# jepsen-io/maelstrom

Hardware: NVIDIA B200
Metric: simulated msgs/sec (broadcast, 4096 nodes) (higher is better)
Workload: dtype int64

## Files before the change

maelstrom_b200/csrc/ms_device.cuh:

```cuda
#pragma once
#include <stdint.h>
#include "../../include/maelstrom_b200.h"

#if defined(__CUDACC__)
#define MS_HD __host__ __device__ __forceinline__
#else
#define MS_HD inline
#endif

namespace msd {

constexpr int64_t  kTickNs   = 1000000;
constexpr uint32_t kInjector = 0xFFFFFFFFu;
constexpr uint8_t  kRemoved  = 0x80;

enum : uint32_t {
  E_NONE = 0, E_RING_OVERFLOW = 1, E_WINDOW_OVERFLOW = 2, E_JOURNAL_OVERFLOW = 3,
  E_INVALID_DEST = 4, E_HISTORY = 5, E_VALUE_RANGE = 6, E_MAIL_OVERFLOW = 7,
  E_CALENDAR_OVERFLOW = 8, E_ID_RANGE = 9, E_BARRIER = 10, E_SNAPSHOT = 11,
  E_RAFT_CAPACITY = 12, E_HISTORY_RING = 13
};

#ifndef MS_CLS0_NT
#define MS_CLS0_NT 64
// ... 53 lines not shown
  uint64_t ev_total, em_total;
};

struct NetParams {
  uint64_t loss_thresh;
  uint64_t exp_coeff;
  uint32_t dist;
  uint32_t mean_ms;
  uint32_t scale;
  uint32_t pair_active;
  uint32_t comp_active;
  uint32_t any_removed;
};

struct Params {
  DevState* st;
  NetParams* np;
  uint8_t*  kind;
  uint32_t* tail;
  uint32_t* limit;
  uint32_t* head;
  uint64_t* ep_born;
  uint4*    ring;
  uint32_t  ring_cap, ring_cap_s;
  uint32_t  n_ep, n_servers, n_inj_tickets, max_window, max_window_s;
  RoundMeta* rmeta;
  uint32_t* rt_em;
  uint32_t* rt_ev;
  uint64_t* rt_chunk;
  uint64_t* rt_cnt;
  uint64_t* phase_cycles;
  uint32_t  n_shards, shard_id;
  uint4*    ring_sh[8];
  uint32_t* tail_sh[8];
  uint32_t* head_sh[8];
  uint64_t* rt_cnt_sh[8];
  uint32_t* bar_sh[8];
  uint32_t  hist, hist_mask, t_max, n_classes;
  uint32_t  split_commit;
  uint64_t* cm_blk;
  uint32_t* cm_flags;
  uint32_t* cls_list;
  uint32_t  cls_cap[4];
  uint4*    jraw;
  uint4*    jbody;
  uint64_t  jmask;
// ... 196 lines not shown
```

maelstrom_b200/csrc/ms_engine.cu:

```cuda
#include <cuda_runtime.h>
#include <math.h>
#include <stdio.h>
#include <stdlib.h>
#include <string.h>

#include <algorithm>
#include <deque>
#include <mutex>
#include <new>
#include <string>
#include <unordered_map>
#include <vector>

#include "ms_device.cuh"
#include "ms_tree.h"
#include "ms_fressian.h"
#include "ms_json.h"

using namespace msd;

extern "C" {
cudaError_t msk_round_smem_attr(size_t bytes);
size_t msk_round_smem_bytes(uint32_t cap);
int msk_round_occupancy(int threads, size_t smem);
// ... 544 lines not shown
  if (cudaGetDeviceCount(&ndev) != cudaSuccess || ndev == 0) {
    set_err("no CUDA device: maelstrom_b200 has no CPU fallback");
    return MS_ERR_CUDA;
  }
  s->device = c.device;
  CK(cudaSetDevice(s->device));
  CK(cudaStreamCreateWithFlags(&s->stream, cudaStreamNonBlocking));
  for (int k = 0; k < 4; k++) CK(cudaStreamCreateWithFlags(&s->aux_streams[k], cudaStreamNonBlocking));
  for (int k = 0; k < 5; k++) CK(cudaEventCreateWithFlags(&s->aux_events[k], cudaEventDisableTiming));

  Params& P = s->P;
  memset(&P, 0, sizeof P);
  const uint32_t M = c.max_endpoints;
  int rc;
  if ((rc = s->dalloc(&P.st, 1))) return rc;
  if ((rc = s->dalloc(&P.np, 1))) return rc;
  if ((rc = s->dalloc(&P.kind, M))) return rc;
  if ((rc = s->dalloc(&P.tail, M))) return rc;
  if ((rc = s->dalloc(&P.limit, M))) return rc;
  if ((rc = s->dalloc(&P.head, M))) return rc;
  if ((rc = s->dalloc(&P.ep_born, M))) return rc;
  {
    void* ptr = nullptr;
    CK(cudaMalloc(&ptr, ((size_t)c.n_nodes * c.server_ring_cap + (size_t)(M - c.n_nodes) * c.ring_cap) * 48));
    s->allocs.push_back(ptr);
    P.ring = (uint4*)ptr;
  }
  P.ring_cap = c.ring_cap;
  P.ring_cap_s = c.server_ring_cap;
  P.n_servers = c.n_nodes;
  P.n_ep = c.n_nodes;
  P.n_inj_tickets = 8;
  P.max_window = c.max_window;
  P.max_window_s = c.server_max_window;
  s->use_graph = c.reserved[1] == 1;
  P.n_shards = c.n_shards;
  P.shard_id = c.shard_id;
  {
    P.t_max = M + P.n_inj_tickets;
    const uint32_t hist = history_rows(c.reserved[0], P.t_max);
    P.hist = hist;
    P.hist_mask = hist - 1;
    if ((rc = s->dalloc(&P.rmeta, hist))) return rc;
    if ((rc = s->dalloc(&P.rt_em, (size_t)hist * P.t_max))) return rc;
    if ((rc = s->dalloc(&P.rt_ev, (size_t)hist * P.t_max))) return rc;
    if ((rc = s->dalloc(&P.rt_chunk, (size_t)hist * P.t_max))) return rc;
    if ((rc = s->dalloc(&P.rt_cnt, (size_t)hist * P.t_max))) return rc;
// ... 1127 lines not shown
  out[0] = (uint64_t)r.state; out[1] = r.term; out[2] = (uint64_t)(r.voted_for + 1); out[3] = r.commit_index;
  out[4] = r.last_applied; out[5] = (uint64_t)(r.leader + 1); out[6] = r.log_size; out[7] = r.kv_size;
  return MS_OK;
}

int ms_counters(ms_sim* s, uint64_t out[8]) {
  std::lock_guard<std::mutex> g(s->mu);
  out[0] = s->hs.rounds_run;
  out[1] = s->hs.stats[2] + s->hs.stats[4];
  out[2] = s->hs.stats[3] + s->hs.stats[5];
  out[3] = s->launches;
  out[4] = s->hs.lost;
  out[5] = s->hs.part_drops;
  out[6] = s->hs.max_window_seen;
  out[7] = s->hs.fallback_sorts;
  return MS_OK;
}

struct ShardBlob {
  uint32_t magic, shard_id, n_shards, t_max;
  uint32_t max_endpoints, ring_cap, hist, pad;
  cudaIpcMemHandle_t ring, tail, head, rt_cnt, bar;
  cudaIpcMemHandle_t gs_snap, gs_tag;
};
static_assert(sizeof(ShardBlob) <= MS_SHARD_BLOB_BYTES, "blob too large");

int ms_shard_handles(ms_sim* s, void* blob_out) {
  std::lock_guard<std::mutex> g(s->mu);
  cudaSetDevice(s->device);
  ShardBlob b;
  memset(&b, 0, sizeof b);
  b.magic = 0x4253534Du;
  b.shard_id = s->P.shard_id; b.n_shards = s->P.n_shards; b.t_max = s->P.t_max;
  b.max_endpoints = s->cfg.max_endpoints; b.ring_cap = s->P.ring_cap ^ (s->P.ring_cap_s << 1); b.hist = s->P.hist;
  CK(cudaIpcGetMemHandle(&b.ring, s->P.ring));
  CK(cudaIpcGetMemHandle(&b.tail, s->P.tail));
  CK(cudaIpcGetMemHandle(&b.head, s->P.head));
  CK(cudaIpcGetMemHandle(&b.rt_cnt, s->P.rt_cnt));
  CK(cudaIpcGetMemHandle(&b.bar, s->P.bar_sh[s->P.shard_id]));
  if (s->P.gs_snap) {
    b.pad = 1;
    CK(cudaIpcGetMemHandle(&b.gs_snap, s->P.gs_snap));
    CK(cudaIpcGetMemHandle(&b.gs_tag, s->P.gs_tag));
  } else if (s->P.rf_heap) {
    b.pad = 2;
    CK(cudaIpcGetMemHandle(&b.gs_snap, s->P.rf_heap));
    CK(cudaIpcGetMemHandle(&b.gs_tag, s->P.rf_ext_off));
  }
  memset(blob_out, 0, MS_SHARD_BLOB_BYTES);
  memcpy(blob_out, &b, sizeof b);
  return MS_OK;
}

int ms_shard_connect(ms_sim* s, uint32_t peer, const void* blob) {
  std::lock_guard<std::mutex> g(s->mu);
  cudaSetDevice(s->device);
  ShardBlob b;
  memcpy(&b, blob, sizeof b);
  if (b.magic != 0x4253534Du || b.shard_id != peer || peer >= s->P.n_shards || b.n_shards != s->P.n_shards ||
      b.t_max != s->P.t_max || b.max_endpoints != s->cfg.max_endpoints || b.ring_cap != (s->P.ring_cap ^ (s->P.ring_cap_s << 1)) ||
      b.hist != s->P.hist) {
    set_err("ms_shard_connect: peer blob does not match this simulation's configuration");
    return MS_ERR_ARG;
  }
  if (peer == s->P.shard_id) return MS_OK;
  void* ptr = nullptr;
  CK(cudaIpcOpenMemHandle(&ptr, b.ring, cudaIpcMemLazyEnablePeerAccess));
  s->peer_ptrs.push_back(ptr); s->P.ring_sh[peer] = (uint4*)ptr;
  CK(cudaIpcOpenMemHandle(&ptr, b.tail, cudaIpcMemLazyEnablePeerAccess));
  s->peer_ptrs.push_back(ptr); s->P.tail_sh[peer] = (uint32_t*)ptr;
  CK(cudaIpcOpenMemHandle(&ptr, b.head, cudaIpcMemLazyEnablePeerAccess));
  s->peer_ptrs.push_back(ptr); s->P.head_sh[peer] = (uint32_t*)ptr;
  CK(cudaIpcOpenMemHandle(&ptr, b.rt_cnt, cudaIpcMemLazyEnablePeerAccess));
  s->peer_ptrs.push_back(ptr); s->P.rt_cnt_sh[peer] = (uint64_t*)ptr;
  CK(cudaIpcOpenMemHandle(&ptr, b.bar, cudaIpcMemLazyEnablePeerAccess));
  s->peer_ptrs.push_back(ptr); s->P.bar_sh[peer] = (uint32_t*)ptr;
  if ((b.pad == 1) != (s->P.gs_snap != nullptr) || (b.pad == 2) != (s->P.rf_heap != nullptr)) {
    set_err("ms_shard_connect: peer runs another workload");
    return MS_ERR_ARG;
  }
  if (b.pad == 2) {
    const size_t N = s->cfg.n_nodes;
    CK(cudaIpcOpenMemHandle(&ptr, b.gs_snap, cudaIpcMemLazyEnablePeerAccess));
    s->peer_ptrs.push_back(ptr); s->P.rf_heap_sh[peer] = (uint4*)ptr;
// ... 100 lines not shown
```

maelstrom_b200/csrc/ms_kernels.cu:

```cuda
#include <cuda_runtime.h>
#include <stdint.h>
#include "ms_device.cuh"

namespace msd {

#define FULL 0xFFFFFFFFu
#ifndef MS_EMUL
#define MS_LAUNCH(kern, grid, block, smem, stream, ...) kern<<<(grid), (block), (smem), (stream)>>>(__VA_ARGS__)
#endif
constexpr int MAXB = 64;
constexpr int MAXNB = 8;
constexpr uint64_t RECV_BIT = 1ull << 63;
constexpr uint32_t kResolvedTicket = 0xFFFFFFu;

__device__ __forceinline__ uint32_t ld_cg_u32(const uint32_t* p) { return __ldcg(p); }
__device__ __forceinline__ void st_v4(uint4* p, uint4 v) {
#ifdef MS_EMUL
  *p = v;
#else
  asm volatile("st.global.L1::no_allocate.v4.u32 [%0], {%1,%2,%3,%4};" ::"l"(p), "r"(v.x), "r"(v.y),
               "r"(v.z), "r"(v.w)
               : "memory");
#endif
}
// ... 23 lines not shown
}

__device__ __forceinline__ bool round_skipped(const Params& p, const DevState* st) {
  if (st->now >= st->stop_ns || st->error) return true;
  if (p.jlevel && !p.jdiscard) {
    const uint64_t raw_base = p.rmeta[(uint32_t)st->round & p.hist_mask].raw_base;
    if (p.n_shards <= 1 && raw_base - st->jraw_drained > ((p.jmask + 1) >> 1)) return true;
    if (st->round - st->drain_round + 2 >= p.hist) return true;
  }
  return false;
}

__device__ __forceinline__ uint32_t slot_tag(uint64_t round) { return 0x80000000u | (uint32_t)(round & 0x7FFFFFFFull); }

struct Rec {
  uint64_t round;
  uint32_t ticket, idx;
  uint32_t src, dest, msg_id, in_reply_to;
  uint32_t tf;
  uint32_t p0;
  uint64_t p1;
};

__device__ __forceinline__ void rec_store(uint4* slot, const Rec& r) {
  st_v4(slot + 0, make_uint4(r.idx, r.ticket, (uint32_t)r.round, (uint32_t)(r.round >> 32)));
  st_v4(slot + 1, make_uint4(r.src, r.dest, r.msg_id, r.in_reply_to));
  st_v4(slot + 2, make_uint4(r.tf, r.p0, (uint32_t)r.p1, (uint32_t)(r.p1 >> 32)));
}
__device__ __forceinline__ Rec rec_unpack(uint4 a, uint4 b, uint4 c) {
  Rec r;
  r.idx = a.x; r.ticket = a.y;
  r.round = (uint64_t)a.z | ((uint64_t)a.w << 32);
  r.src = b.x; r.dest = b.y; r.msg_id = b.z; r.in_reply_to = b.w;
  r.tf = c.x; r.p0 = c.y;
  r.p1 = (uint64_t)c.z | ((uint64_t)c.w << 32);
  return r;
}

__device__ __forceinline__ uint32_t ring_cap_of(const Params& p, uint32_t e) { return e < p.n_servers ? p.ring_cap_s : p.ring_cap; }
__device__ __forceinline__ size_t ring_base(const Params& p, uint32_t e) {
  return e < p.n_servers ? (size_t)e * p.ring_cap_s
                         : (size_t)p.n_servers * p.ring_cap_s + (size_t)(e - p.n_servers) * p.ring_cap;
}
__device__ __forceinline__ uint4* ring_slot(const Params& p, uint4* ring, uint32_t e, uint32_t pos) {
  return ring + (ring_base(p, e) + (pos & (ring_cap_of(p, e) - 1u))) * 3;
}

__device__ __forceinline__ uint64_t dense_base(const Params& p, DevState* st, uint64_t round, uint32_t ticket) {
  if (ticket == kResolvedTicket) return round << 32;
  const uint32_t row = (uint32_t)round & p.hist_mask;
  const RoundMeta* m = p.rmeta + row;
  if (m->round != round || ticket >= p.t_max) {
    latch_error(st, E_HISTORY, (uint32_t)round);
    return 0;
  }
  return m->id_base + p.rt_em[(size_t)row * p.t_max + ticket];
}

__device__ uint64_t block_excl_scan(uint64_t* a, int n, uint64_t* wtmp ) {
  const int nt = blockDim.x, tid = threadIdx.x, lane = tid & 31, warp = tid >> 5;
  const int c = (n + nt - 1) / nt;
  const int lo = min(tid * c, n), hi = min(lo + c, n);
  uint64_t sum = 0;
  for (int i = lo; i < hi; i++) sum += a[i];
  uint64_t incl = sum;
#pragma unroll
  for (int d = 1; d < 32; d <<= 1) {
    const uint64_t y = __shfl_up_sync(FULL, incl, d);
// ... 130 lines not shown
  const int lane = threadIdx.x & 31;
  bool push = false, wheel = false;
  uint32_t wslot = 0;
  const bool undeliverable = valid && (r.dest >= p.n_ep || r.src >= p.n_ep ||
                                       (np.any_removed && ((p.kind[r.dest] | p.kind[r.src]) & kRemoved)));
  if (valid) {
    r.round = cx.round; r.ticket = cx.ticket; r.idx = local_idx;
    uint32_t x[4] = {0xFFFFFFFFu, 0, 0, 0};
    if (cx.need_rng)
      philox4x32_10(local_idx + cx.idx_bias, cx.emitter, (uint32_t)cx.round, (uint32_t)(cx.round >> 32),
                    p.seed_lo, p.seed_hi, x);
    const bool cl = (r.src >= p.n_servers && r.src < p.n_ep && kind_is_client(p.kind[r.src])) ||
                    (r.dest >= p.n_servers && r.dest < p.n_ep && kind_is_client(p.kind[r.dest]));
    const uint64_t lat = cl ? 0ull : (cx.need_rng ? latency_ms(np, x) : cx.const_lat);
    journal_raw(p, cx.chunk + cx.n_recv + local_idx, local_idx, false, r);
    if (cl) cx.c_send_cl++; else cx.c_send_sv++;
    if (undeliverable) {
      atomicAdd((unsigned long long*)&st->undeliverable, 1ull);
    } else if ((uint64_t)x[0] < np.loss_thresh) {
      cx.c_lost++;
    } else if (lat == 0) {
      cx.c_zero++;
      if (has_direct) {
        uint4* ring_o = p.ring_sh[owner_of(r.dest, p.n_servers, p.n_shards)];
        rec_store(ring_slot(p, ring_o, r.dest, direct_pos), r);
      } else {
        push = true;
      }
    } else {
      const uint64_t tick = (uint64_t)(cx.now / kTickNs) + lat;
      const uint64_t laps = (lat - 1) / p.cal_slots;
      if (p.cal == nullptr || laps > 0xFFFFu) {
        latch_error(st, E_CALENDAR_OVERFLOW, (uint32_t)lat);
      } else {
        wheel = true;
        wslot = (uint32_t)tick & (p.cal_slots - 1);
        r.round |= laps << 48;
      }
    }
  }
  if (__any_sync(FULL, wheel)) wheel_file(p, st, wheel, wslot, r);
  if (!__any_sync(FULL, push)) return;
  const uint32_t key = push ? r.dest : (0x80000000u | (uint32_t)lane);
  const uint32_t mask = __match_any_sync(FULL, key);
  const int leader = __ffs(mask) - 1;
  const uint32_t rank = __popc(mask & ((1u << lane) - 1u));
  uint32_t base = 0;
  const uint32_t o = push ? owner_of(r.dest, p.n_servers, p.n_shards) : 0u;
  if (push && lane == leader) base = atomicAdd(&p.tail_sh[o][r.dest], (uint32_t)__popc(mask));
  base = __shfl_sync(FULL, base, leader);
  if (push) {
    const uint32_t pos = base + rank;
    if ((uint32_t)(pos - p.head_sh[o][r.dest]) >= ring_cap_of(p, r.dest)) {
      latch_error(st, E_RING_OVERFLOW, r.dest);
    } else {
      rec_store(ring_slot(p, p.ring_sh[o], r.dest, pos), r);
    }
  }
}

__global__ void k_set_bit(uint32_t* words, size_t word, uint32_t bit) { atomicOr(words + word, 1u << bit); }

__device__ __forceinline__ void gen_hist(const Params& p, DevState* st, int64_t now, uint64_t round, uint32_t e,
                                         const GenDev& g, uint32_t op, uint32_t type, uint32_t f, uint32_t error, uint32_t value) {
  const unsigned long long pos = atomicAdd((unsigned long long*)&st->gc_hist_n, 1ull);
  if (pos - st->gc_hist_drained > p.gc_hist_mask) { latch_error(st, E_HISTORY_RING, e); return; }
  uint4* at = p.gc_hist + (pos & p.gc_hist_mask) * 2;
  const uint64_t order = (round << 24) | g.ordinal;
  at[0] = make_uint4((uint32_t)now, (uint32_t)((uint64_t)now >> 32), (uint32_t)order, (uint32_t)(order >> 32));
  at[1] = make_uint4(e, op, type | (f << 8) | (error << 16), value);
}

__device__ __forceinline__ bool gen_timer_due(const Params& p, const GenDev& g, int64_t now) {
  if (g.waiting_for) return now >= g.deadline_ns;
  if (g.phase == GEN_MIX) return now >= p.gc_limit_ns || now >= g.next_op_ns;
  if (g.phase == GEN_QUIET) return now >= p.gc_limit_ns + p.gc_quiet_ns;
  return g.phase == GEN_FINAL;
}

__device__ bool gen_step(const Params& p, DevState* st, uint32_t e, int64_t now, uint64_t round, const uint4* myring,
                         uint32_t head, uint32_t my_mask, uint32_t n, const uint16_t* ord, const uint32_t* vals, Rec& out) {
  GenDev g = p.gc[e];
  for (uint32_t pos = 0; pos < n; pos++) {
    const uint32_t i = ord[pos];
    if (!(vals[i] & (1u << 30))) continue;
    const uint4* rp = myring + (size_t)((head + i) & my_mask) * 3;
    const uint4 vb = rp[1], vc = rp[2];
    const uint32_t type = vc.x & 0xFFFFu, flags = vc.x >> 16;
    if (!g.waiting_for || !(flags & MS_F_REPLY) || vb.w != g.waiting_for) continue;
    uint32_t outcome = MS_H_OK, err = 0, value = g.cur_value;
    if (type == MS_T_ERROR) {
      err = vc.y;
      const bool definite = err != 0 && err != 13;
      outcome = (definite || g.cur_f == MS_HF_READ) ? MS_H_FAIL : MS_H_INFO;
    } else if (g.cur_f == MS_HF_READ) {
      value = vc.y;
    }
    gen_hist(p, st, now, round, e, g, g.ops, outcome, g.cur_f, err, value);
    g.waiting_for = 0;
  }
  if (g.waiting_for && now >= g.deadline_ns) {
    gen_hist(p, st, now, round, e, g, g.ops, g.cur_f == MS_HF_READ ? MS_H_FAIL : MS_H_INFO, g.cur_f, MS_H_TIMEOUT, g.cur_value);
    g.waiting_for = 0;
  }
  bool send = false;
  if (!g.waiting_for) {
    uint32_t f = MS_HF_READ, value = 0;
    if (g.phase == GEN_MIX) {
      if (now >= p.gc_limit_ns) g.phase = GEN_QUIET;
      else if (now >= g.next_op_ns) {
        uint32_t x[4];
        philox4x32_10(g.ops, e, 0xC11E47u, 0u, p.seed_lo, p.seed_hi, x);
        if ((((uint64_t)x[0] * 1000u) >> 32) >= p.gc_read_permille) { f = MS_HF_BROADCAST; value = g.ordinal + p.gc_n * g.bcasts++; }
        g.next_op_ns = now + (int64_t)(((unsigned __int128)x[1] * (unsigned __int128)(2 * (uint64_t)p.gc_interval_ns)) >> 32);
        send = true;
      }
    }
    if (g.phase == GEN_QUIET && now >= p.gc_limit_ns + p.gc_quiet_ns) { g.phase = GEN_FINAL; send = true; }
    else if (g.phase == GEN_FINAL && !send) g.phase = GEN_DONE;
// ... 158 lines not shown
    }
    const bool again = valid && laps > 0;
    if (__any_sync(FULL, again)) {
      Rec r = rec_unpack(a, b, c);
      r.round = (r.round & 0xFFFFFFFFFFFFull) | ((uint64_t)(laps - 1u) << 48);
      wheel_file(p, st, again, slot, r);
    }
    if (again) valid = false;
    const uint32_t dest = b.y;
    if (valid && (((uint64_t)a.x | ((uint64_t)a.z << 32)) < p.ep_born[dest])) valid = false;
    const uint32_t key = valid ? dest : (0x80000000u | (uint32_t)lane);
    const uint32_t mask = __match_any_sync(FULL, key);
    const int leader = __ffs(mask) - 1;
    const uint32_t rank = __popc(mask & ((1u << lane) - 1u));
    uint32_t base = 0;
    const uint32_t o = valid ? owner_of(dest, p.n_servers, p.n_shards) : 0u;
    if (valid && lane == leader) base = atomicAdd(&p.tail_sh[o][dest], (uint32_t)__popc(mask));
    base = __shfl_sync(FULL, base, leader);
    if (valid) {
      const uint32_t pos = base + rank;
      if ((uint32_t)(pos - p.head_sh[o][dest]) >= ring_cap_of(p, dest)) {
        latch_error(st, E_RING_OVERFLOW, dest);
      } else {
        uint4* dst = ring_slot(p, p.ring_sh[o], dest, pos);
        st_v4(dst, a); st_v4(dst + 1, b); st_v4(dst + 2, c);
      }
    }
  }
}

struct MsgView {
  uint32_t src, msg_id, p0;
  uint32_t tf;
};

__device__ __forceinline__ MsgView view_load(const uint4* rec) {
  const uint4 b = rec[1], c = rec[2];
  MsgView v;
  v.src = b.x; v.msg_id = b.z; v.tf = c.x; v.p0 = c.y;
  return v;
}

constexpr uint32_t V_FRESH = 1u << 31;
constexpr uint32_t V_RECV = 1u << 30;
constexpr uint32_t V_CAND = 1u << 29;
constexpr uint32_t V_MASK = (1u << 29) - 1u;


struct NbrList {
  const uint32_t* nl;
  uint32_t deg;
};

__device__ __forceinline__ uint32_t nbr_count(const Params& p, uint32_t e) {
  if (p.topology == MS_TOPO_TOTAL) return p.n_servers - 1;
  return p.nbr_off[e + 1] - p.nbr_off[e];
}
__device__ __forceinline__ uint32_t nbr_at(const Params& p, uint32_t e, uint32_t j) {
  if (p.topology == MS_TOPO_TOTAL) return j < e ? j : j + 1;
  return p.nbr[p.nbr_off[e] + j];
}
__device__ __forceinline__ uint32_t nbr_pos(const Params& p, uint32_t e, uint32_t src) {
  if (p.topology == MS_TOPO_TOTAL) {
    if (src >= p.n_servers || src == e) return 0xFFFFFFFFu;
// ... 664 lines not shown
      if (valid) {
        const uint32_t g = lo + j;
        if (g < n_host) {
          const ms_msg m = p.inj_buf[g];
          r.src = m.src; r.dest = m.dest; r.msg_id = m.msg_id; r.in_reply_to = m.in_reply_to;
          r.tf = (uint32_t)m.type | ((uint32_t)m.flags << 16); r.p0 = m.p0; r.p1 = m.p1;
        } else {
          const ms_op op = p.sched[cur + (g - n_host)];
          r.src = op.src; r.dest = op.dest; r.msg_id = op.body.msg_id; r.in_reply_to = op.body.in_reply_to;
          r.tf = (uint32_t)op.body.type | ((uint32_t)op.body.flags << 16); r.p0 = op.body.p0; r.p1 = op.body.p1;
        }
      }
      emit_one(p, st, np, cx, valid, r, j, 0, false);
    }
  } else {
    const uint32_t e = ticket - p.n_inj_tickets;
    const uint8_t kind = p.kind[e];
    const uint32_t head = p.head[e];
    uint32_t n = ((kind & kRemoved)) ? 0u : (p.limit[e] - head);
    if (n > cap || n > (e < p.n_servers ? p.max_window_s : p.max_window)) {
      if (tid == 0) latch_error(st, E_WINDOW_OVERFLOW, e);
      n = 0;
    }
    const uint4* myring = p.ring + ring_base(p, e) * 3;
    const uint32_t my_mask = ring_cap_of(p, e) - 1u;
    const bool is_server = (kind == MS_KIND_SERVER);
    const bool bcast = !GS && is_server && p.workload == MS_W_BROADCAST;
    uint32_t n_timer = 0, fire_seq = 0, fire_p0 = 0;
    if constexpr (GS) {
      if (is_server && p.gs_init[e] && now >= p.gs_next_fire[e]) {
        n_timer = p.n_servers - 1;
        fire_seq = p.gs_fires[e] + 1;
      }
    }
    const uint32_t* mybits = (is_server && p.bitmap) ? p.bitmap + (size_t)e * p.bm_words : nullptr;
    const uint32_t deg = bcast ? nbr_count(p, e) : 0;
    const bool nb_smem = bcast && p.topology != MS_TOPO_TOTAL && deg <= MAXNB;
    if (nb_smem && tid < (int)deg) s_nbr[tid] = p.nbr[p.nbr_off[e] + tid];
    __syncthreads();

    {
      uint32_t err_val = 0xFFFFFFFFu;
      uint32_t snap_gone = 0xFFFFFFFFu;
      bool inj_srv = false;
      const bool nb4 = nb_smem && deg <= 4;
      const uint32_t nr0 = (nb4 && deg > 0) ? s_nbr[0] : 0xFFFFFFFFu, nr1 = (nb4 && deg > 1) ? s_nbr[1] : 0xFFFFFFFFu;
      const uint32_t nr2 = (nb4 && deg > 2) ? s_nbr[2] : 0xFFFFFFFFu, nr3 = (nb4 && deg > 3) ? s_nbr[3] : 0xFFFFFFFFu;
      for (int base = 0; base < (int)n; base += 2 * nt) {
        uint4 a[2], b[2], c[2];
#pragma unroll
        for (int q = 0; q < 2; q++) {
          const int i = base + q * nt + tid;
          if (i < (int)n) {
            const uint4* rp = myring + (size_t)((head + i) & my_mask) * 3;
            a[q] = rp[0]; b[q] = rp[1]; c[q] = rp[2];
          }
        }
#pragma unroll
        for (int q = 0; q < 2; q++) {
          const int i = base + q * nt + tid;
          if (i >= (int)n) continue;
          const uint64_t rnd = (uint64_t)a[q].z | ((uint64_t)a[q].w << 32);
          keyA[i] = (rnd << 24) | (uint64_t)(a[q].y & 0xFFFFFFu);
          keyB[i] = a[q].x;
          const uint32_t src = b[q].x, tf = c[q].x, v = c[q].y;
          if (a[q].y < p.n_inj_tickets && src < p.n_servers) inj_srv = true;
          bool cut = false;
          if (np.pair_active && p.pair_bits)
            cut = (p.pair_bits[(size_t)e * p.pair_words + (src >> 5)] >> (src & 31)) & 1u;
          if (!cut && np.comp_active) {
            const uint32_t cs = p.comp[src], ce = p.comp[e];
            cut = cs != ce && cs != 0xFFFFFFFFu && ce != 0xFFFFFFFFu;
          }
          const uint32_t type = tf & 0xFFFFu;
          const uint32_t fl = tf >> 16;
          uint32_t tc = TC_OTHER;
          if constexpr (GS) {
            if (type == MS_T_INIT) tc = GT_INIT;
            else if (type == MS_T_ADD) tc = GT_ADD;
            else if (type == MS_T_READ) tc = GT_READ;
            else if (type == MS_T_REPLICATE_ONE) tc = GT_REPL_ONE;
            else if (type == MS_T_REPLICATE_FULL) tc = GT_REPL_FULL;
          } else {
          if (type == MS_T_INIT) tc = TC_INIT;
          else if (type == MS_T_TOPOLOGY) tc = TC_TOPOLOGY;
          else if (type == MS_T_READ) tc = TC_READ;
          else if (type == MS_T_BROADCAST) tc = TC_BROADCAST;
          else if (type == MS_T_ECHO) tc = TC_ECHO;
          }
          uint32_t slot = 0;
          if (nb4) {
            slot = src == nr3 ? 4u : src == nr2 ? 3u : src == nr1 ? 2u : src == nr0 ? 1u : 0u;
          } else if (nb_smem) {
            for (uint32_t j = 0; j < deg; j++) if (s_nbr[j] == src) slot = j + 1;
          } else if (bcast && src < p.n_servers && src != e) {
            slot = 15;
          }
          meta[i] = (uint16_t)(slot | ((fl & MS_F_MSG_ID) ? M_HAS_ID : 0u) | ((fl & MS_F_REPLY) ? M_REPLY : 0u) |
                               (tc << M_TC_SHIFT));
          uint32_t val = cut ? 0u : V_RECV;
          if (bcast && !cut && tc == TC_BROADCAST && !(fl & MS_F_REPLY)) {
            if (v >= p.n_values || v > V_MASK) err_val = v;
            else val |= v | V_CAND;
          }
          if constexpr (GS) {
            if (is_server && !cut && !(fl & MS_F_REPLY)) {
              if (tc == GT_ADD || tc == GT_REPL_ONE) {
                if (v >= p.n_values || v > V_MASK) err_val = v;
                else val |= v;
              } else if (tc == GT_REPL_FULL) {
                const uint32_t run = c[q].z;
                const uint32_t rowi = src * p.gs_slots + (run & (p.gs_slots - 1));
                if (src >= p.n_servers ||
                    __ldcg(p.gs_tag_sh[owner_of(src, p.n_servers, p.n_shards)] + rowi) != run) snap_gone = src;
                else val |= rowi;
              }
            }
          }
          vals[i] = val;
        }
      }
      if (err_val != 0xFFFFFFFFu) latch_error(st, E_VALUE_RANGE, err_val);
      if (snap_gone != 0xFFFFFFFFu) latch_error(st, E_SNAPSHOT, snap_gone);
      if (inj_srv) s_misc[3] = 1;
    }
    if (bcast) {
      for (int base = 0; base < (int)n; base += 4 * nt) {
        uint32_t w[4], vv[4];
#pragma unroll
        for (int q = 0; q < 4; q++) {
          const int i = base + q * nt + tid;
          vv[q] = i < (int)n ? vals[i] : 0u;
          w[q] = (vv[q] & V_CAND) ? mybits[(vv[q] & V_MASK) >> 5] : 0xFFFFFFFFu;
        }
#pragma unroll
        for (int q = 0; q < 4; q++) {
          const int i = base + q * nt + tid;
          if (i < (int)n && (vv[q] & V_CAND) && !((w[q] >> (vv[q] & 31)) & 1u)) vals[i] = vv[q] | V_FRESH;
        }
      }
    }
    __syncthreads();
    PHASE_MARK(1);
    if (tid == 0 && next_li < my_count) {
      const uint32_t t2 = next_li < my_big ? my_list[next_li] : my_list[p.t_max - 1u - (next_li - my_big)];
      if (t2 >= p.n_inj_tickets) {
        const uint32_t e2 = t2 - p.n_inj_tickets;
        const uint32_t h2 = p.head[e2], n2 = p.limit[e2] - h2, cap2 = ring_cap_of(p, e2);
        if (n2 > 0 && n2 <= cap2) {
          const uint4* base2 = p.ring + ring_base(p, e2) * 3;
          const uint32_t o2 = h2 & (cap2 - 1u), first = min(n2, cap2 - o2);
          prefetch_l2_bulk(base2 + (size_t)o2 * 3, first * 48u);
          if (n2 > first) prefetch_l2_bulk(base2, (n2 - first) * 48u);
        }
      }
    }

    uint32_t R = 0;
    bool use_blocks = false;
    if (n > 0) {
      const int c = ((int)n + nt - 1) / nt;
      const int lo = min(tid * c, (int)n), hi = min(lo + c, (int)n);
      uint32_t nf = 0;
      uint32_t fmask = 0;
      const bool use_mask = c <= 32;
      if (lo < hi) {
        uint64_t pa = lo ? keyA[lo - 1] : 0ull;
        uint32_t pb = lo ? keyB[lo - 1] : 0u;
        for (int i = lo; i < hi; i++) {
          const uint64_t ka = keyA[i];
          const uint32_t kb = keyB[i];
          if (i == 0 || ka != pa || kb <= pb) { nf++; fmask |= 1u << ((i - lo) & 31); }
          pa = ka; pb = kb;
        }
      }
      uint32_t off = block_excl_scan_u32(nf, &R, s_wcnt);
// ... 106 lines not shown
            if ((vals[ord[cur]] & V_MASK) == v) {
              while ((uint32_t)pos < cur) {
                const uint32_t old = atomicCAS(&tab[h], (unsigned short)cur, (unsigned short)pos);
                if (old == cur) break;
                cur = old;
              }
              break;
            }
            h = (h + 1) & (tsz - 1);
          }
        }
      }
      __syncthreads();
    }
    if constexpr (RF) {
      if (is_server) {
        if (tid == 0) {
          RaftCtx c{p, st, e, now, round, p.rf_node + e, p.rf_log + (size_t)e * p.rf_log_cap * 2,
                    p.rf_cb + (size_t)e * (p.rf_cb_mask + 1u) * 2, p.rf_stage + (size_t)e * p.rf_stage_cap * 3, 0u, 0u, 0u, 0u};
          rf_group_of(p, e, c.gbase, c.gn);
          for (uint32_t pos = 0; pos < n; pos++) {
            const uint32_t i = ord[pos];
            if (!(vals[i] & V_RECV)) continue;
            const uint4* rp = myring + (size_t)((head + i) & my_mask) * 3;
            if (p.workload == MS_W_RAFT) rf_handle(c, rec_unpack(rp[0], rp[1], rp[2]));
            else if (p.workload == MS_W_TXN_TREE) tt_handle(c, rec_unpack(rp[0], rp[1], rp[2]));
            else txn_handle(c, rec_unpack(rp[0], rp[1], rp[2]));
          }
          if (p.workload == MS_W_RAFT) { rf_actions(c); rf_note_busy(c); }
          if (p.workload == MS_W_TXN_TREE) tt_actions(c);
          s_misc[2] = c.n_stage;
        }
        __syncthreads();
        n_timer = s_misc[2];
      }
    }
    if (kind == MS_KIND_GEN_CLIENT) {
      if (tid == 0) {
        Rec q;
        const bool send = gen_step(p, st, e, now, round, myring, head, my_mask, n, ord, vals, q);
        if (send) {
          s_gen[0] = make_uint4(q.src, q.dest, q.msg_id, q.in_reply_to);
          s_gen[1] = make_uint4(q.tf, q.p0, 0u, 0u);
        }
        s_misc[2] = send ? 1u : 0u;
      }
      __syncthreads();
      n_timer = s_misc[2];
    }
    if constexpr (SV) {
      if (kind == MS_KIND_SERVICE) {
        uint32_t* skey = reinterpret_cast<uint32_t*>(tab);
        for (uint32_t pos = tid; pos < n; pos += nt) {
          const uint32_t i = ord[pos];
          const uint4* rp = myring + (size_t)((head + i) & my_mask) * 3;
          const uint4 vc = rp[2];
          reg1[pos] = (uint64_t)vc.z | ((uint64_t)vc.w << 32);
          skey[pos] = vc.y;
          const uint32_t ty = vc.x & 0xFFFFu;
          meta[i] = (uint16_t)((ty < 0xFFu ? ty : 0xFFu) | ((vc.x >> 8) & 0xFF00u));
        }
        __syncthreads();
        if (tid == 0) {
          uint32_t svc = 0;
          while (svc < 4 && p.sv_ep[svc] != e) svc++;
          uint32_t n_rep = 0;
          uint32_t ck = 0xFFFFFFFFu, cval = 0;
          bool chas = false, cdirty = false;
          for (uint32_t pos = 0; pos < n && svc < 4; pos++) {
            const uint32_t i = ord[pos];
            if (!(vals[i] & V_RECV)) continue;
            SvReq q;
            q.type = meta[i] & 0xFFu; q.flags = meta[i] >> 8; q.key = skey[pos];
            q.p1 = reg1[pos];
            q.src = 0;
            if (svc == MS_SVC_SEQ_KV)
              q.src = (myring + (size_t)((head + i) & my_mask) * 3)[1].x;
            const bool keyed = q.type == MS_T_READ || q.type == MS_T_WRITE || q.type == MS_T_CAS;
            if (svc != MS_SVC_LIN_TSO && keyed && q.key >= p.sv_n_keys) { latch_error(st, E_VALUE_RANGE, q.key); continue; }
            if (svc != MS_SVC_LIN_TSO && !keyed) continue;
            uint32_t x[4] = {0, 0, 0, 0};
            if (svc == MS_SVC_SEQ_KV || svc == MS_SVC_LWW_KV)
              philox4x32_10(n_rep, e, (uint32_t)round, (uint32_t)(round >> 32), p.seed_lo, p.seed_hi, x);
            SvRep r;
            if (svc == MS_SVC_LIN_KV) {
              r.reply = false; r.otype = MS_T_ERROR; r.code = 0; r.value = 0;
              if (keyed) {
                if (q.key != ck) {
                  if (cdirty) { p.sv_lin_has[ck] = chas ? 1 : 0; p.sv_lin_val[ck] = cval; }
                  ck = q.key; chas = p.sv_lin_has[ck] != 0; cval = p.sv_lin_val[ck]; cdirty = false;
                }
                bool np_; uint32_t nv;
                kv_eval(chas, cval, q, false, r, np_, nv);
                if (r.reply) { cdirty = cdirty || np_ != chas || nv != cval; chas = np_; cval = nv; }
              }
            } else {
              service_handle(p, svc, q, x[3], r);
            }
            if (r.reply) {
              vals[i] |= SV_REPLY | (r.code << 16) | r.otype;
// ... 181 lines not shown
      s_nbbase[tid] = base;
    }
    __syncthreads();
    cx.chunk = s_chunk;
    cx.n_recv = n_recv;
    cx.emitter = e;
    const bool cl_ep = kind_is_client(kind);
    const uint32_t msg_id_base = (is_server && p.next_msg_id) ? p.next_msg_id[e] : 0;
    const uint32_t set_before = (is_server && p.set_count) ? p.set_count[e] : 0;
    NbrList L;
    L.nl = nb_smem ? s_nbr : nullptr;
    L.deg = deg;
    PHASE_MARK(5);

    const bool full_recv = p.jlevel >= 2 || mailed || !use_blocks;
    for (uint32_t pos = tid; pos < n; pos += nt) {
      const uint32_t i = ord[pos];
      const uint32_t val = vals[i];
      if (!(val & V_RECV)) { c_part++; continue; }
      const uint32_t k = (uint32_t)(aux[pos] >> 32) & 0xFFFFu;
      const uint32_t mt = meta[i];
      const uint32_t sslot = mt & M_SRCSLOT;
      if (full_recv || !nb_smem || sslot == 0) {
        const uint4* rp = myring + (size_t)((head + i) & my_mask) * 3;
        Rec m = rec_unpack(rp[0], rp[1], rp[2]);
        const uint64_t id = (use_blocks ? s_bbase[blk[pos]] : dense_base(p, st, m.round, m.ticket)) + m.idx;
        journal_raw(p, cx.chunk + k, id, true, m);
        const bool cl = cl_ep || (m.src >= p.n_servers && kind_is_client(p.kind[m.src]));
        if (cl) c_recv_cl++; else c_recv_sv++;
        if (kind == MS_KIND_SIM_CLIENT && ((m.tf >> 16) & MS_F_REPLY)) c_replies++;
        if (mailed) {
          const uint32_t mpos = s_misc[0] + k;
          if (mpos >= p.mail_cap) {
            latch_error(st, E_MAIL_OVERFLOW, e);
          } else {
            uint4* dst = reinterpret_cast<uint4*>(p.mail) + (size_t)mpos * 3;
            st_v4(dst + 0, make_uint4((uint32_t)id, (uint32_t)(id >> 32), (uint32_t)now, (uint32_t)((uint64_t)now >> 32)));
            st_v4(dst + 1, make_uint4(m.src, m.dest, m.msg_id, m.in_reply_to));
            st_v4(dst + 2, make_uint4(m.tf, m.p0, (uint32_t)m.p1, (uint32_t)(m.p1 >> 32)));
          }
        }
      } else {
        const uint64_t id = s_bbase[blk[pos]] + keyB[i];
        const uint64_t vrec = id | RECV_BIT;
        if (p.jlevel)
          st_v4(p.jraw + ((cx.chunk + k) & p.jmask),
                make_uint4((uint32_t)vrec, (uint32_t)(vrec >> 32), s_nbr[sslot - 1], e));
        c_recv_sv++;
// ... 52 lines not shown
        const uint32_t k = jm - (uint32_t)a0;
        const uint32_t my_emit = (uint32_t)aux[pos + 1] - (uint32_t)a0;
        const uint32_t new_before = (uint32_t)(a0 >> 48);
        const uint32_t i = ord[pos];
        const uint32_t val = vals[i];
        const uint32_t mt = meta[i];
        const bool gossip = bcast && ((mt >> M_TC_SHIFT) & 7u) == TC_BROADCAST && !(mt & M_REPLY) &&
                            !((mt & M_HAS_ID) && k == my_emit - 1);
        if (gossip && nb_smem) {
          const uint32_t ss = mt & M_SRCSLOT;
          const uint32_t js = (ss && k >= ss - 1) ? k + 1 : k;
          r.dest = s_nbr[js];
          r.msg_id = 0; r.in_reply_to = 0; r.tf = MS_T_BROADCAST; r.p0 = val & V_MASK; r.p1 = 0;
          if (agg_mode == 1) {
            direct = s_nbbase[js] + new_before - s_S[blk[pos]][js];
            has_direct = true;
          } else if (agg_mode == 2) {
            const uint32_t f = js < 2 ? (F01[pos] >> (16 * js)) : (F23[pos] >> (16 * (js - 2)));
            direct = s_nbbase[js] + new_before - (f & 0xFFFFu);
            has_direct = true;
          }
          fast = has_direct && !np.any_removed;
        } else {
          const uint4* rp = myring + (size_t)((head + i) & my_mask) * 3;
          const uint4 vb = rp[1], vc = rp[2];
          MsgView w;
          w.src = vb.x; w.msg_id = vb.z; w.tf = vc.x; w.p0 = vc.y;
          const uint64_t p1 = (uint64_t)vc.z | ((uint64_t)vc.w << 32);
          bool svc_emission = false;
          if constexpr (SV) {
            if (kind == MS_KIND_SERVICE) {
              svc_emission = true;
              r.src = e; r.dest = w.src; r.msg_id = 0; r.in_reply_to = w.msg_id;
              r.tf = (val & 0xFFFFu) | ((uint32_t)MS_F_REPLY << 16);
              r.p0 = (val >> 16) & 0xFFu;
              r.p1 = keyB[pos];
            }
          }
          if (svc_emission) {
          } else if constexpr (GS) {
            const uint32_t tc = (mt >> M_TC_SHIFT) & 7u;
            r.src = e; r.dest = w.src; r.msg_id = 0; r.in_reply_to = w.msg_id; r.p0 = 0; r.p1 = 0;
            uint32_t otype = MS_T_ERROR;
            if (tc == GT_INIT) otype = MS_T_INIT_OK;
            else if (tc == GT_ADD) otype = MS_T_ADD_OK;
            else if (tc == GT_READ) { otype = MS_T_READ_OK; r.p0 = keyB[pos]; }
            else r.p0 = 10;
            r.tf = otype | ((uint32_t)MS_F_REPLY << 16);
          } else {
          (void)node_emit(p, e, w, k, my_emit, jm, msg_id_base, set_before, new_before, p1, r, L);
          }
        }
      }
      if (fast) {
        r.round = round; r.ticket = ticket; r.idx = j;
        journal_raw(p, cx.chunk + n_recv + j, j, false, r);
        cx.c_send_sv++;
        cx.c_zero++;
        uint4* ring_o = p.ring_sh[owner_of(r.dest, p.n_servers, p.n_shards)];
        rec_store(ring_o + ((size_t)r.dest * p.ring_cap_s + (direct & (p.ring_cap_s - 1u))) * 3, r);
      }
      if (__any_sync(FULL, valid && !fast)) emit_one(p, st, np, cx, valid && !fast, r, j, direct, has_direct);
    }
    if (tid == 0 && is_server) {
      if (p.workload == MS_W_ECHO && p.next_msg_id && n_emit) p.next_msg_id[e] = msg_id_base + n_emit;
      if constexpr (!GS) {
      if (p.set_count && n_new) p.set_count[e] = set_before + n_new;
      } else {
        int64_t nf = p.gs_next_fire[e];
        if (n_timer) {
          nf += (int64_t)p.gs_interval_ms * kTickNs;
          p.gs_fires[e] = fire_seq;
          p.gs_tag[e * p.gs_slots + (fire_seq & (p.gs_slots - 1))] = fire_seq;
        }
        if (s_misc[2]) { p.gs_init[e] = 1; nf = now; }
        p.gs_next_fire[e] = nf;
      }
      if (n > st->max_window_seen) atomicMax(&st->max_window_seen, n);
    }
  }

  PHASE_MARK(6);
  {
// ... 366 lines not shown
```

Before: 12.52 billion.

## Split ring records into key and body arrays, compact gossip records

Ring storage changes from interleaved 48-byte records to a struct-of-arrays layout: a 16-byte key array followed by a 32-byte body array. Zero-latency broadcast gossip writes only a compact 16-byte key record whose flag bit marks it, and readers rebuild the full message from ticket, round low bits and value. Ingest and prefetch read only keys on the broadcast fast path, which cuts memory traffic per delivered message. The cost is extra branching on the compact flag and reconstructing the round from its low 32 bits, which assumes records never span more than 2^32 rounds.

```diff
diff --git a/maelstrom_b200/csrc/ms_device.cuh b/maelstrom_b200/csrc/ms_device.cuh
--- a/maelstrom_b200/csrc/ms_device.cuh
+++ b/maelstrom_b200/csrc/ms_device.cuh
@@ -99,6 +99,7 @@
   uint32_t* head;
   uint64_t* ep_born;
   uint4*    ring;
+  uint64_t  ring_slots;
   uint32_t  ring_cap, ring_cap_s;
   uint32_t  n_ep, n_servers, n_inj_tickets, max_window, max_window_s;
   RoundMeta* rmeta;
diff --git a/maelstrom_b200/csrc/ms_engine.cu b/maelstrom_b200/csrc/ms_engine.cu
--- a/maelstrom_b200/csrc/ms_engine.cu
+++ b/maelstrom_b200/csrc/ms_engine.cu
@@ -590,7 +590,8 @@
   if ((rc = s->dalloc(&P.ep_born, M))) return rc;
   {
     void* ptr = nullptr;
-    CK(cudaMalloc(&ptr, ((size_t)c.n_nodes * c.server_ring_cap + (size_t)(M - c.n_nodes) * c.ring_cap) * 48));
+    P.ring_slots = (size_t)c.n_nodes * c.server_ring_cap + (size_t)(M - c.n_nodes) * c.ring_cap;
+    CK(cudaMalloc(&ptr, P.ring_slots * 48));
     s->allocs.push_back(ptr);
     P.ring = (uint4*)ptr;
   }
@@ -1764,6 +1765,7 @@
   uint32_t max_endpoints, ring_cap, hist, pad;
   cudaIpcMemHandle_t ring, tail, head, rt_cnt, bar;
   cudaIpcMemHandle_t gs_snap, gs_tag;
+  uint64_t ring_slots;
 };
 static_assert(sizeof(ShardBlob) <= MS_SHARD_BLOB_BYTES, "blob too large");
 
@@ -1775,6 +1777,7 @@
   b.magic = 0x4253534Du;
   b.shard_id = s->P.shard_id; b.n_shards = s->P.n_shards; b.t_max = s->P.t_max;
   b.max_endpoints = s->cfg.max_endpoints; b.ring_cap = s->P.ring_cap ^ (s->P.ring_cap_s << 1); b.hist = s->P.hist;
+  b.ring_slots = s->P.ring_slots;
   CK(cudaIpcGetMemHandle(&b.ring, s->P.ring));
   CK(cudaIpcGetMemHandle(&b.tail, s->P.tail));
   CK(cudaIpcGetMemHandle(&b.head, s->P.head));
@@ -1801,7 +1804,7 @@
   memcpy(&b, blob, sizeof b);
   if (b.magic != 0x4253534Du || b.shard_id != peer || peer >= s->P.n_shards || b.n_shards != s->P.n_shards ||
       b.t_max != s->P.t_max || b.max_endpoints != s->cfg.max_endpoints || b.ring_cap != (s->P.ring_cap ^ (s->P.ring_cap_s << 1)) ||
-      b.hist != s->P.hist) {
+      b.hist != s->P.hist || b.ring_slots != s->P.ring_slots) {
     set_err("ms_shard_connect: peer blob does not match this simulation's configuration");
     return MS_ERR_ARG;
   }
diff --git a/maelstrom_b200/csrc/ms_kernels.cu b/maelstrom_b200/csrc/ms_kernels.cu
--- a/maelstrom_b200/csrc/ms_kernels.cu
+++ b/maelstrom_b200/csrc/ms_kernels.cu
@@ -69,10 +69,15 @@
   uint64_t p1;
 };
 
+__device__ __forceinline__ void rec_pack(const Rec& r, uint4& a, uint4& b, uint4& c) {
+  a = make_uint4(r.idx, r.ticket, (uint32_t)r.round, (uint32_t)(r.round >> 32));
+  b = make_uint4(r.src, r.dest, r.msg_id, r.in_reply_to);
+  c = make_uint4(r.tf, r.p0, (uint32_t)r.p1, (uint32_t)(r.p1 >> 32));
+}
 __device__ __forceinline__ void rec_store(uint4* slot, const Rec& r) {
-  st_v4(slot + 0, make_uint4(r.idx, r.ticket, (uint32_t)r.round, (uint32_t)(r.round >> 32)));
-  st_v4(slot + 1, make_uint4(r.src, r.dest, r.msg_id, r.in_reply_to));
-  st_v4(slot + 2, make_uint4(r.tf, r.p0, (uint32_t)r.p1, (uint32_t)(r.p1 >> 32)));
+  uint4 a, b, c;
+  rec_pack(r, a, b, c);
+  st_v4(slot + 0, a); st_v4(slot + 1, b); st_v4(slot + 2, c);
 }
 __device__ __forceinline__ Rec rec_unpack(uint4 a, uint4 b, uint4 c) {
   Rec r;
@@ -89,8 +94,40 @@
   return e < p.n_servers ? (size_t)e * p.ring_cap_s
                          : (size_t)p.n_servers * p.ring_cap_s + (size_t)(e - p.n_servers) * p.ring_cap;
 }
-__device__ __forceinline__ uint4* ring_slot(const Params& p, uint4* ring, uint32_t e, uint32_t pos) {
-  return ring + (ring_base(p, e) + (pos & (ring_cap_of(p, e) - 1u))) * 3;
+__device__ __forceinline__ size_t ring_index(const Params& p, uint32_t e, uint32_t pos) {
+  return ring_base(p, e) + (pos & (ring_cap_of(p, e) - 1u));
+}
+__device__ __forceinline__ void ring_put(const Params& p, uint4* ring, size_t g, uint4 a, uint4 b, uint4 c) {
+  uint4* body = ring + p.ring_slots + 2 * g;
+  st_v4(ring + g, a); st_v4(body, b); st_v4(body + 1, c);
+}
+__device__ __forceinline__ void ring_store(const Params& p, uint4* ring, uint32_t e, uint32_t pos, const Rec& r) {
+  uint4 a, b, c;
+  rec_pack(r, a, b, c);
+  ring_put(p, ring, ring_index(p, e, pos), a, b, c);
+}
+constexpr uint32_t kCompact = 1u << 31;
+__device__ __forceinline__ void ring_store_gossip(uint4* ring, size_t g, uint32_t idx, uint32_t ticket, uint64_t round,
+                                                  uint32_t value) {
+  st_v4(ring + g, make_uint4(idx, ticket | kCompact, (uint32_t)round, value));
+}
+__device__ __forceinline__ uint64_t compact_round(uint64_t cur, uint32_t lo) { return cur - (uint32_t)((uint32_t)cur - lo); }
+__device__ __forceinline__ Rec ring_expand(const Params& p, uint4 a, uint4 b, uint4 c, uint64_t cur, uint32_t owner) {
+  if (!(a.y & kCompact)) return rec_unpack(a, b, c);
+  Rec r;
+  r.idx = a.x; r.ticket = a.y & 0xFFFFFFu;
+  r.round = compact_round(cur, a.z);
+  r.src = r.ticket - p.n_inj_tickets; r.dest = owner; r.msg_id = 0; r.in_reply_to = 0;
+  r.tf = MS_T_BROADCAST; r.p0 = a.w; r.p1 = 0;
+  return r;
+}
+__device__ __forceinline__ Rec ring_load(const Params& p, const uint4* ring, size_t g, uint64_t cur, uint32_t owner) {
+  const uint4* body = ring + p.ring_slots + 2 * g;
+  return ring_expand(p, ring[g], body[0], body[1], cur, owner);
+}
+__device__ __forceinline__ Rec ring_load_body(const Params& p, const uint4* ring, size_t g) {
+  const uint4* body = ring + p.ring_slots + 2 * g;
+  return rec_unpack(make_uint4(0u, 0u, 0u, 0u), body[0], body[1]);
 }
 
 __device__ __forceinline__ uint64_t dense_base(const Params& p, DevState* st, uint64_t round, uint32_t ticket) {
@@ -267,8 +304,7 @@
     } else if (lat == 0) {
       cx.c_zero++;
       if (has_direct) {
-        uint4* ring_o = p.ring_sh[owner_of(r.dest, p.n_servers, p.n_shards)];
-        rec_store(ring_slot(p, ring_o, r.dest, direct_pos), r);
+        ring_store(p, p.ring_sh[owner_of(r.dest, p.n_servers, p.n_shards)], r.dest, direct_pos, r);
       } else {
         push = true;
       }
@@ -299,7 +335,7 @@
     if ((uint32_t)(pos - p.head_sh[o][r.dest]) >= ring_cap_of(p, r.dest)) {
       latch_error(st, E_RING_OVERFLOW, r.dest);
     } else {
-      rec_store(ring_slot(p, p.ring_sh[o], r.dest, pos), r);
+      ring_store(p, p.ring_sh[o], r.dest, pos, r);
     }
   }
 }
@@ -323,23 +359,22 @@
   return g.phase == GEN_FINAL;
 }
 
-__device__ bool gen_step(const Params& p, DevState* st, uint32_t e, int64_t now, uint64_t round, const uint4* myring,
+__device__ bool gen_step(const Params& p, DevState* st, uint32_t e, int64_t now, uint64_t round, size_t my0,
                          uint32_t head, uint32_t my_mask, uint32_t n, const uint16_t* ord, const uint32_t* vals, Rec& out) {
   GenDev g = p.gc[e];
   for (uint32_t pos = 0; pos < n; pos++) {
     const uint32_t i = ord[pos];
     if (!(vals[i] & (1u << 30))) continue;
-    const uint4* rp = myring + (size_t)((head + i) & my_mask) * 3;
-    const uint4 vb = rp[1], vc = rp[2];
-    const uint32_t type = vc.x & 0xFFFFu, flags = vc.x >> 16;
-    if (!g.waiting_for || !(flags & MS_F_REPLY) || vb.w != g.waiting_for) continue;
+    const Rec m = ring_load_body(p, p.ring, my0 + ((head + i) & my_mask));
+    const uint32_t type = m.tf & 0xFFFFu, flags = m.tf >> 16;
+    if (!g.waiting_for || !(flags & MS_F_REPLY) || m.in_reply_to != g.waiting_for) continue;
     uint32_t outcome = MS_H_OK, err = 0, value = g.cur_value;
     if (type == MS_T_ERROR) {
-      err = vc.y;
+      err = m.p0;
       const bool definite = err != 0 && err != 13;
       outcome = (definite || g.cur_f == MS_HF_READ) ? MS_H_FAIL : MS_H_INFO;
     } else if (g.cur_f == MS_HF_READ) {
-      value = vc.y;
+      value = m.p0;
     }
     gen_hist(p, st, now, round, e, g, g.ops, outcome, g.cur_f, err, value);
     g.waiting_for = 0;
@@ -544,8 +579,7 @@
       if ((uint32_t)(pos - p.head_sh[o][dest]) >= ring_cap_of(p, dest)) {
         latch_error(st, E_RING_OVERFLOW, dest);
       } else {
-        uint4* dst = ring_slot(p, p.ring_sh[o], dest, pos);
-        st_v4(dst, a); st_v4(dst + 1, b); st_v4(dst + 2, c);
+        ring_put(p, p.ring_sh[o], ring_index(p, dest, pos), a, b, c);
       }
     }
   }
@@ -555,13 +589,6 @@
   uint32_t src, msg_id, p0;
   uint32_t tf;
 };
-
-__device__ __forceinline__ MsgView view_load(const uint4* rec) {
-  const uint4 b = rec[1], c = rec[2];
-  MsgView v;
-  v.src = b.x; v.msg_id = b.z; v.tf = c.x; v.p0 = c.y;
-  return v;
-}
 
 constexpr uint32_t V_FRESH = 1u << 31;
 constexpr uint32_t V_RECV = 1u << 30;
@@ -1272,7 +1299,7 @@
       if (tid == 0) latch_error(st, E_WINDOW_OVERFLOW, e);
       n = 0;
     }
-    const uint4* myring = p.ring + ring_base(p, e) * 3;
+    const size_t my0 = ring_base(p, e);
     const uint32_t my_mask = ring_cap_of(p, e) - 1u;
     const bool is_server = (kind == MS_KIND_SERVER);
     const bool bcast = !GS && is_server && p.workload == MS_W_BROADCAST;
@@ -1296,25 +1323,47 @@
       const bool nb4 = nb_smem && deg <= 4;
       const uint32_t nr0 = (nb4 && deg > 0) ? s_nbr[0] : 0xFFFFFFFFu, nr1 = (nb4 && deg > 1) ? s_nbr[1] : 0xFFFFFFFFu;
       const uint32_t nr2 = (nb4 && deg > 2) ? s_nbr[2] : 0xFFFFFFFFu, nr3 = (nb4 && deg > 3) ? s_nbr[3] : 0xFFFFFFFFu;
+      const uint4* body = p.ring + p.ring_slots;
+      const bool keys_first = bcast && !need_rng && const_lat == 0;
       for (int base = 0; base < (int)n; base += 2 * nt) {
-        uint4 a[2], b[2], c[2];
+        uint4 a[2];
+        uint32_t q_src[2], q_tf[2], q_v[2], q_run[2];
 #pragma unroll
         for (int q = 0; q < 2; q++) {
           const int i = base + q * nt + tid;
           if (i < (int)n) {
-            const uint4* rp = myring + (size_t)((head + i) & my_mask) * 3;
-            a[q] = rp[0]; b[q] = rp[1]; c[q] = rp[2];
+            const size_t g = my0 + ((head + i) & my_mask);
+            a[q] = p.ring[g];
+            if (!keys_first) {
+              const uint4 b = body[2 * g], c = body[2 * g + 1];
+              q_src[q] = b.x; q_tf[q] = c.x; q_v[q] = c.y; q_run[q] = c.z;
+            }
+          }
+        }
+        if (bcast) {
+#pragma unroll
+          for (int q = 0; q < 2; q++) {
+            const int i = base + q * nt + tid;
+            if (i >= (int)n) continue;
+            if (a[q].y & kCompact) {
+              q_src[q] = (a[q].y & 0xFFFFFFu) - p.n_inj_tickets; q_tf[q] = MS_T_BROADCAST; q_v[q] = a[q].w; q_run[q] = 0;
+            } else if (keys_first) {
+              const size_t g = my0 + ((head + i) & my_mask);
+              const uint4 b = body[2 * g], c = body[2 * g + 1];
+              q_src[q] = b.x; q_tf[q] = c.x; q_v[q] = c.y; q_run[q] = c.z;
+            }
           }
         }
 #pragma unroll
         for (int q = 0; q < 2; q++) {
           const int i = base + q * nt + tid;
           if (i >= (int)n) continue;
-          const uint64_t rnd = (uint64_t)a[q].z | ((uint64_t)a[q].w << 32);
-          keyA[i] = (rnd << 24) | (uint64_t)(a[q].y & 0xFFFFFFu);
+          const uint32_t tk = a[q].y & 0xFFFFFFu;
+          const uint64_t rnd = (a[q].y & kCompact) ? compact_round(round, a[q].z) : ((uint64_t)a[q].z | ((uint64_t)a[q].w << 32));
+          keyA[i] = (rnd << 24) | (uint64_t)tk;
           keyB[i] = a[q].x;
-          const uint32_t src = b[q].x, tf = c[q].x, v = c[q].y;
-          if (a[q].y < p.n_inj_tickets && src < p.n_servers) inj_srv = true;
+          const uint32_t src = q_src[q], tf = q_tf[q], v = q_v[q];
+          if (tk < p.n_inj_tickets && src < p.n_servers) inj_srv = true;
           bool cut = false;
           if (np.pair_active && p.pair_bits)
             cut = (p.pair_bits[(size_t)e * p.pair_words + (src >> 5)] >> (src & 31)) & 1u;
@@ -1359,7 +1408,7 @@
                 if (v >= p.n_values || v > V_MASK) err_val = v;
                 else val |= v;
               } else if (tc == GT_REPL_FULL) {
-                const uint32_t run = c[q].z;
+                const uint32_t run = q_run[q];
                 const uint32_t rowi = src * p.gs_slots + (run & (p.gs_slots - 1));
                 if (src >= p.n_servers ||
                     __ldcg(p.gs_tag_sh[owner_of(src, p.n_servers, p.n_shards)] + rowi) != run) snap_gone = src;
@@ -1398,10 +1447,15 @@
         const uint32_t e2 = t2 - p.n_inj_tickets;
         const uint32_t h2 = p.head[e2], n2 = p.limit[e2] - h2, cap2 = ring_cap_of(p, e2);
         if (n2 > 0 && n2 <= cap2) {
-          const uint4* base2 = p.ring + ring_base(p, e2) * 3;
+          const size_t g2 = ring_base(p, e2);
           const uint32_t o2 = h2 & (cap2 - 1u), first = min(n2, cap2 - o2);
-          prefetch_l2_bulk(base2 + (size_t)o2 * 3, first * 48u);
-          if (n2 > first) prefetch_l2_bulk(base2, (n2 - first) * 48u);
+          prefetch_l2_bulk(p.ring + g2 + o2, first * 16u);
+          if (n2 > first) prefetch_l2_bulk(p.ring + g2, (n2 - first) * 16u);
+          if (GS || need_rng || const_lat != 0 || p.workload != MS_W_BROADCAST || p.kind[e2] != MS_KIND_SERVER) {
+            const uint4* body2 = p.ring + p.ring_slots + 2 * g2;
+            prefetch_l2_bulk(body2 + 2 * (size_t)o2, first * 32u);
+            if (n2 > first) prefetch_l2_bulk(body2, (n2 - first) * 32u);
+          }
         }
       }
     }
@@ -1554,10 +1608,10 @@
           for (uint32_t pos = 0; pos < n; pos++) {
             const uint32_t i = ord[pos];
             if (!(vals[i] & V_RECV)) continue;
-            const uint4* rp = myring + (size_t)((head + i) & my_mask) * 3;
-            if (p.workload == MS_W_RAFT) rf_handle(c, rec_unpack(rp[0], rp[1], rp[2]));
-            else if (p.workload == MS_W_TXN_TREE) tt_handle(c, rec_unpack(rp[0], rp[1], rp[2]));
-            else txn_handle(c, rec_unpack(rp[0], rp[1], rp[2]));
+            const Rec m = ring_load(p, p.ring, my0 + ((head + i) & my_mask), round, e);
+            if (p.workload == MS_W_RAFT) rf_handle(c, m);
+            else if (p.workload == MS_W_TXN_TREE) tt_handle(c, m);
+            else txn_handle(c, m);
           }
           if (p.workload == MS_W_RAFT) { rf_actions(c); rf_note_busy(c); }
           if (p.workload == MS_W_TXN_TREE) tt_actions(c);
@@ -1570,7 +1624,7 @@
     if (kind == MS_KIND_GEN_CLIENT) {
       if (tid == 0) {
         Rec q;
-        const bool send = gen_step(p, st, e, now, round, myring, head, my_mask, n, ord, vals, q);
+        const bool send = gen_step(p, st, e, now, round, my0, head, my_mask, n, ord, vals, q);
         if (send) {
           s_gen[0] = make_uint4(q.src, q.dest, q.msg_id, q.in_reply_to);
           s_gen[1] = make_uint4(q.tf, q.p0, 0u, 0u);
@@ -1585,12 +1639,11 @@
         uint32_t* skey = reinterpret_cast<uint32_t*>(tab);
         for (uint32_t pos = tid; pos < n; pos += nt) {
           const uint32_t i = ord[pos];
-          const uint4* rp = myring + (size_t)((head + i) & my_mask) * 3;
-          const uint4 vc = rp[2];
-          reg1[pos] = (uint64_t)vc.z | ((uint64_t)vc.w << 32);
-          skey[pos] = vc.y;
-          const uint32_t ty = vc.x & 0xFFFFu;
-          meta[i] = (uint16_t)((ty < 0xFFu ? ty : 0xFFu) | ((vc.x >> 8) & 0xFF00u));
+          const Rec m = ring_load_body(p, p.ring, my0 + ((head + i) & my_mask));
+          reg1[pos] = m.p1;
+          skey[pos] = m.p0;
+          const uint32_t ty = m.tf & 0xFFFFu;
+          meta[i] = (uint16_t)((ty < 0xFFu ? ty : 0xFFu) | ((m.tf >> 8) & 0xFF00u));
         }
         __syncthreads();
         if (tid == 0) {
@@ -1607,7 +1660,7 @@
             q.p1 = reg1[pos];
             q.src = 0;
             if (svc == MS_SVC_SEQ_KV)
-              q.src = (myring + (size_t)((head + i) & my_mask) * 3)[1].x;
+              q.src = ring_load_body(p, p.ring, my0 + ((head + i) & my_mask)).src;
             const bool keyed = q.type == MS_T_READ || q.type == MS_T_WRITE || q.type == MS_T_CAS;
             if (svc != MS_SVC_LIN_TSO && keyed && q.key >= p.sv_n_keys) { latch_error(st, E_VALUE_RANGE, q.key); continue; }
             if (svc != MS_SVC_LIN_TSO && !keyed) continue;
@@ -1835,8 +1888,7 @@
       const uint32_t mt = meta[i];
       const uint32_t sslot = mt & M_SRCSLOT;
       if (full_recv || !nb_smem || sslot == 0) {
-        const uint4* rp = myring + (size_t)((head + i) & my_mask) * 3;
-        Rec m = rec_unpack(rp[0], rp[1], rp[2]);
+        const Rec m = ring_load(p, p.ring, my0 + ((head + i) & my_mask), round, e);
         const uint64_t id = (use_blocks ? s_bbase[blk[pos]] : dense_base(p, st, m.round, m.ticket)) + m.idx;
         journal_raw(p, cx.chunk + k, id, true, m);
         const bool cl = cl_ep || (m.src >= p.n_servers && kind_is_client(p.kind[m.src]));
@@ -1935,11 +1987,11 @@
           }
           fast = has_direct && !np.any_removed;
         } else {
-          const uint4* rp = myring + (size_t)((head + i) & my_mask) * 3;
-          const uint4 vb = rp[1], vc = rp[2];
+          const size_t g = my0 + ((head + i) & my_mask);
+          const Rec m = bcast ? ring_load(p, p.ring, g, round, e) : ring_load_body(p, p.ring, g);
           MsgView w;
-          w.src = vb.x; w.msg_id = vb.z; w.tf = vc.x; w.p0 = vc.y;
-          const uint64_t p1 = (uint64_t)vc.z | ((uint64_t)vc.w << 32);
+          w.src = m.src; w.msg_id = m.msg_id; w.tf = m.tf; w.p0 = m.p0;
+          const uint64_t p1 = m.p1;
           bool svc_emission = false;
           if constexpr (SV) {
             if (kind == MS_KIND_SERVICE) {
@@ -1966,12 +2018,11 @@
         }
       }
       if (fast) {
-        r.round = round; r.ticket = ticket; r.idx = j;
         journal_raw(p, cx.chunk + n_recv + j, j, false, r);
         cx.c_send_sv++;
         cx.c_zero++;
-        uint4* ring_o = p.ring_sh[owner_of(r.dest, p.n_servers, p.n_shards)];
-        rec_store(ring_o + ((size_t)r.dest * p.ring_cap_s + (direct & (p.ring_cap_s - 1u))) * 3, r);
+        ring_store_gossip(p.ring_sh[owner_of(r.dest, p.n_servers, p.n_shards)],
+                          (size_t)r.dest * p.ring_cap_s + (direct & (p.ring_cap_s - 1u)), j, ticket, round, r.p0);
       }
       if (__any_sync(FULL, valid && !fast)) emit_one(p, st, np, cx, valid && !fast, r, j, direct, has_direct);
     }
```

New measurement: 13.99 billion, median of 6. 11.7% higher.
